# epfl-lts2/pygsp

Hardware: AMD Instinct MI355X
Metric: filtered-vertices/sec (N·Nsig·K/s) + achieved HBM GB/s vs roofline, 1M-vertex K=30 (higher is better)
Workload: dtype f64

## Files before the change

pygsp_amd/csrc/gspx.hip:

```cpp
#include "gspx_kernels.hip.h"
#include "gspx_tile_kernels.hip.h"

#include <hip/hip_runtime.h>

#include <algorithm>
#include <atomic>
#include <chrono>
#include <cmath>
#include <cstdarg>
#include <cstdio>
#include <cstring>
#include <map>
#include <memory>
#include <numeric>
#include <mutex>
#include <string>
#include <thread>
#include <vector>
#include <sys/mman.h>

#include "../../include/gspx.h"
#include "../../include/gspx_ext.h"

using namespace gspx;
// ... 292 lines not shown
  int64_t tile_pad = 1;
  int64_t tile_min_row = 16;
  int64_t staged_copy = 1;
  int64_t staged_copy_min_mb = 32;
  int64_t copy_threads = 0;
  int64_t tile_regroup = 1;
  int64_t tile_lg = 0;
  int64_t edge_vertex_walk = 1;
  int64_t fuse_input = 1;
  int64_t tile_nt = -1;
  int64_t synthesis = 0;
  int64_t alternate_sweep = 1;
  int64_t xcd_remap = 1;
  int64_t combine = 0;
  int64_t ws_limit_mb = 65536;
  int64_t max_batch = 0;
  int64_t gather_rccl = 1;
  int64_t lds_pad_kb = 0;
  int64_t host_pipeline = 1;
  int64_t host_batch = 0;
  int64_t host_edge = 0;
  int64_t host_threads = 0;
  int64_t streamed_alloc = 1;
};

struct gspx_ctx {
  int device = 0;
  int cu_count = 256;
  hipStream_t stream = nullptr;
  Options opt;
  DevMem ws_t;
  DevMem ws_r;
  DevMem ws_w;
  DevMem io_x, io_y;
  DevMem ws_spec;
  DevMem ws_sq, ws_sqp;
  HostPipe* pipe = nullptr;
  CopyStage* copy = nullptr;
  bool counted = false;
  std::mutex comms_mu;
  std::vector<struct gspx_comm*> comms;
  hipEvent_t ev[4] = {nullptr, nullptr, nullptr, nullptr};
  std::vector<hipEvent_t> ev_pool;
  double timing[8] = {0, 0, 0, 0, 0, 0, 0, 0};
  bool capturing = false;
  std::vector<unsigned char> seen_key;
  std::vector<unsigned char> graph_key;
  hipGraphExec_t graph_exec = nullptr;
};

static std::atomic<int> g_live_ctx[64];

static void replay_reset(gspx_ctx* ctx) {
  if (!ctx) return;
  ctx->seen_key.clear();
  ctx->graph_key.clear();
  if (ctx->graph_exec) {
    (void)hipGraphExecDestroy(ctx->graph_exec);
    ctx->graph_exec = nullptr;
  }
}

struct gspx_buf {
  gspx_ctx* ctx = nullptr;
  DevMem mem;
  int64_t bytes = 0;
// ... 86 lines not shown
    ctx->cu_count = 256;
  hipError_t e = hipStreamCreateWithFlags(&ctx->stream, hipStreamNonBlocking);
  if (e != hipSuccess) {
    delete ctx;
    return set_err(GSPX_ERR_HIP, "hipStreamCreate failed: %s", hipGetErrorString(e));
  }
  for (int i = 0; i < 4; ++i) {
    e = hipEventCreate(&ctx->ev[i]);
    if (e != hipSuccess) {
      delete ctx;
      return set_err(GSPX_ERR_HIP, "hipEventCreate failed: %s", hipGetErrorString(e));
    }
  }
  *out = ctx;
  return GSPX_OK;
}

static void comm_invalidate_all(gspx_ctx* ctx);

extern "C" int gspx_ctx_destroy(gspx_ctx* ctx) {
  replay_reset(ctx);
  if (!ctx) return GSPX_OK;
  if (ctx->counted) g_live_ctx[ctx->device & 63].fetch_sub(1);
  comm_invalidate_all(ctx);
  if (ctx->graph_exec) {
    (void)hipGraphExecDestroy(ctx->graph_exec);
    ctx->graph_exec = nullptr;
  }
  (void)hipSetDevice(ctx->device);
  if (ctx->stream) (void)hipStreamSynchronize(ctx->stream);
  for (int i = 0; i < 4; ++i)
    if (ctx->ev[i]) (void)hipEventDestroy(ctx->ev[i]);
  for (hipEvent_t e : ctx->ev_pool) (void)hipEventDestroy(e);
  ctx->ws_t.release();
  ctx->ws_r.release();
  ctx->ws_w.release();
  ctx->io_x.release();
  ctx->io_y.release();
  ctx->ws_spec.release();
  ctx->ws_sq.release();
  ctx->ws_sqp.release();
  if (ctx->pipe) {
    ctx->pipe->destroy();
    delete ctx->pipe;
    ctx->pipe = nullptr;
  }
  if (ctx->copy) {
    ctx->copy->destroy();
    delete ctx->copy;
    ctx->copy = nullptr;
  }
  if (ctx->stream) (void)hipStreamDestroy(ctx->stream);
  delete ctx;
  return GSPX_OK;
}

extern "C" int gspx_ctx_sync(gspx_ctx* ctx) {
  if (!ctx) return set_err(GSPX_ERR_INVALID, "null ctx");
  HIPCHK(hipSetDevice(ctx->device));
  HIPCHK(hipStreamSynchronize(ctx->stream));
  return GSPX_OK;
}

static int64_t* option_slot(Options& o, const char* key) {
  if (!key) return nullptr;
  if (!strcmp(key, "kernel")) return &o.kernel;
// ... 1039 lines not shown
}
static int sqnorm_gx(const gspx_ctx* ctx, int N, unsigned w) {
  const int cwl = sqnorm_cwl(w);
  const int64_t tiles = ((int64_t)N + (64 >> cwl) - 1) / (64 >> cwl);
  const int64_t gy = ((int64_t)w + (1 << cwl) - 1) >> cwl;
  return (int)std::max<int64_t>(1, std::min<int64_t>(tiles, (4 * (int64_t)ctx->cu_count + gy - 1) / gy));
}
static size_t sqnorm_parts(const gspx_ctx* ctx, int N, unsigned w) {
  return (size_t)sqnorm_gx(ctx, N, w) * SQ_PASS * w;
}

template <typename T>
static int launch_combine_sqnorm(gspx_ctx* ctx, const T* slots, int nslots, size_t slot_stride, unsigned pitch, int N,
                                 unsigned w, const SqNorms& sq, hipStream_t st) {
  const size_t lds = (size_t)nslots * 64 * sizeof(double);
  const int cwl = sqnorm_cwl(w);
  const dim3 grid((unsigned)sqnorm_gx(ctx, N, w), (w + (1u << cwl) - 1) >> cwl);
  for (int f0 = 0; f0 < sq.nf; f0 += SQ_PASS) {
    const int here = std::min(SQ_PASS, sq.nf - f0);
    const int fb = here <= 8 ? 2 : here <= 32 ? 8 : 32;
    typedef void (*kern_t)(const T*, int, size_t, u32, int, int, int, const double*, int, double*);
    const kern_t kern = fb == 2 ? k_combine_sqnorm<T, 2> : fb == 8 ? k_combine_sqnorm<T, 8> : k_combine_sqnorm<T, 32>;
    if (lds > ((size_t)64 << 10))
      HIPCHK(hipFuncSetAttribute((const void*)kern, hipFuncAttributeMaxDynamicSharedMemorySize, (int)lds));
    hipLaunchKernelGGL(kern, grid, dim3(256), lds, st, slots, nslots, slot_stride, (u32)pitch, N, (int)w, cwl,
                       sq.cf + f0, sq.ldc, sq.part);
    const int64_t n = (int64_t)here * w;
    hipLaunchKernelGGL(k_sqnorm_reduce, dim3((unsigned)((n + 255) / 256)), dim3(256), 0, st, sq.part, (int)grid.x,
                       4 * fb, here, (int)w, sq.out + (size_t)f0 * sq.ldo, sq.ldo);
  }
  return GSPX_OK;
}

template <typename T> static int ensure_factor(gspx_graph* g, double lmax) {
  if (g->fval_lmax == lmax) return GSPX_OK;
  gspx_ctx* ctx = g->ctx;
  const int N = (int)g->N;
  const T a1 = (T)(lmax / 2.0), a2 = (T)(lmax / 2.0);
  const T two_over_a1 = T(2) / a1;
  const int nb = std::max(1, (N + 255) / 256);
  if (N > 0)
    hipLaunchKernelGGL((k_factor<T>), dim3(nb), dim3(256), 0, ctx->stream, g->rptr.as<int>(),
                       g->rcol.as<int>(), g->rval.as<T>(), N, two_over_a1, a2, g->fval.as<T>());
  HIPCHK(hipGetLastError());
  g->fval_lmax = lmax;
  return GSPX_OK;
}

static hipEvent_t pool_event(gspx_ctx* ctx, size_t& i_ref) {
  size_t i = i_ref - 1;
  if (i >= 1024) {
    i = 1020 + (i & 3);
    i_ref = i + 1;
  }
  while (ctx->ev_pool.size() <= i) {
    hipEvent_t e = nullptr;
    if (hipEventCreate(&e) != hipSuccess) return nullptr;
    ctx->ev_pool.push_back(e);
  }
  return ctx->ev_pool[i];
}

__global__ void k_s1nat(const int* __restrict__ s1, const int* __restrict__ perm, int n, int* __restrict__ nat) {
  const int i = blockIdx.x * 256 + threadIdx.x;
  if (i < n) nat[i] = perm[s1[i]];
}
// ... 162 lines not shown
  a.perm = g->has_perm ? g->perm.as<int>() : nullptr;
  return a;
}

static int batch_events(gspx_ctx* ctx, size_t& ev_idx, hipEvent_t ev[4]) {
  for (int i = 0; i < 4; ++i) ev[i] = pool_event(ctx, ++ev_idx);
  if (!ev[0] || !ev[1] || !ev[2] || !ev[3]) return set_err(GSPX_ERR_HIP, "hipEventCreate failed");
  HIPCHK(hipEventRecord(ev[0], ctx->stream));
  return GSPX_OK;
}

template <typename T>
static int run_batch(gspx_graph* g, int nf, int M, const std::vector<double>& cp, const T* x,
                     unsigned ldx, T* y, unsigned ldy, unsigned ld, bool deferred,
                     bool acc_existing, bool final_to_y, size_t& ev_idx, const SqNorms* sq = nullptr) {
  gspx_ctx* ctx = g->ctx;
  const Options& opt = ctx->opt;
  hipStream_t st = ctx->stream;
  const int N = (int)g->N;
  const int K = M - 1;
  const WorkPanels wp = work_panels<T>(g, opt, deferred || nf == 1, 1, ld, y, ldy);
  const bool tile_direct = wp.tile_direct, padded = wp.padded;
  const unsigned ldw = wp.ldw;
  const size_t U = (size_t)N * ldw;
  const Shape shape = choose_shape(opt, sizeof(T), ld, vec_cap(4, ldy, y));
  const int* perm = g->has_perm ? g->perm.as<int>() : nullptr;

  std::vector<PlanStep> plan;
  if (deferred)
    make_plan_deferred(nf, M, plan);
  else
    make_plan_fused(nf, M, cp, acc_existing, final_to_y, plan);

  std::vector<T> hw;
  if (deferred) {
    hw.resize((size_t)nf * M);
    for (size_t i = 0; i < hw.size(); ++i) hw[i] = (T)cp[i];
  } else {
    hw.resize((size_t)K * nf * 3);
    for (int k = 0; k < K; ++k)
      for (int j = 0; j < nf * 3; ++j) hw[(size_t)k * nf * 3 + j] = (T)plan[(size_t)k].w[(size_t)j];
  }
  const bool cap = ctx->capturing;
  if (!cap) {
    CHK(ctx->ws_w.ensure(hw.size() * sizeof(T) + 64));
    HIPCHK(hipMemcpyAsync(ctx->ws_w.p, hw.data(), hw.size() * sizeof(T), hipMemcpyHostToDevice, st));
    HIPCHK(hipStreamSynchronize(st));
  }

  const size_t nslots = deferred ? (size_t)M : 2;
  const size_t SU = U;
  CHK(ctx->ws_t.ensure(nslots * SU * sizeof(T) + 256));
  if (!deferred) CHK(ctx->ws_r.ensure((size_t)nf * U * sizeof(T) + 256));
  T* slots = ctx->ws_t.as<T>();
  T* racc = ctx->ws_r.as<T>();

  hipEvent_t ev[4] = {};
  if (!cap) CHK(batch_events(ctx, ev_idx, ev));
  const bool tile_ok = tile_direct || padded;
  const unsigned char* xb = (const unsigned char*)x;
  const unsigned char* yb = (const unsigned char*)y;
  const size_t xbytes = (size_t)N * ldx * sizeof(T), ybytes = (size_t)nf * N * ldy * sizeof(T);
  const bool fuse_in = tile_direct && !deferred && opt.fuse_input && g->gt_slow == 0 && ldx == ld &&
                       ((uintptr_t)x % 16) == 0 && (xb + xbytes <= yb || yb + ybytes <= xb) &&
                       (!g->has_perm || (g->gt_ns1 > 0 && (!cap || g->gt_s1nat.p)));
  if (fuse_in) {
    CHK(ensure_s1nat(g, st));
  } else if (padded) {
    const unsigned nb = (unsigned)std::min<size_t>((U + 255) / 256, 65536);
    hipLaunchKernelGGL((k_permute_in_pad<T>), dim3(nb), dim3(256), 0, st, x, ldx, slots, ldw, ld, N, perm);
  } else {
    launch_permute_in<T>(x, ldx, slots, ld, N, perm, vec_cap(shape.vec, ldx, x), st);
  }
  if (!cap) HIPCHK(hipEventRecord(ev[1], st));

  CHK(prepare_coff<T>(g, shape, ld, st));
  StepArgs<T> a = step_base<T>(g, ld, y, ldy);
  a.nf = nf;
  a.racc = racc;
  for (int k = 1; k <= K; ++k) {
    const PlanStep& ps = plan[(size_t)k - 1];
    if (tile_ok) {
      TileArgs<T> t{};
      if (deferred) {
        t.cur = slots + (size_t)(k - 1) * SU;
        t.old = (k >= 2 && ps.gamma != 0.0) ? slots + (size_t)(k - 2) * SU : t.cur;
        t.out = slots + (size_t)k * SU;
      } else {
        t.cur = slots + (size_t)((k - 1) & 1) * SU;
        t.old = ps.gamma == 0.0 ? t.cur : slots + (size_t)(k & 1) * SU;
        t.out = slots + (size_t)(k & 1) * SU;
        if (fuse_in && k == 1) {
          t.cur = x;
          t.old = x;
          t.s1rows = g->has_perm ? g->gt_s1nat.as<int>() : nullptr;
        } else if (fuse_in && k == 2) {
          t.old = x;
          t.old_rows = perm;
        }
      }
      t.racc = racc;
      t.y = y;
      t.ldy = ldy;
      t.perm = perm;
      t.scale = (T)ps.scale;
      t.gamma = (T)ps.gamma;
      t.beta = T(0);
      t.flush = ps.flush;
      t.final = padded ? 0 : ps.final;
      t.reverse = (opt.alternate_sweep && (k & 1)) ? 1 : 0;
      if (ps.flush) {
        t.wn = (T)ps.w[0];
        t.wc = (T)ps.w[1];
        t.wo = (T)ps.w[2];
      }
      CHK(launch_step_tile<T>(g, opt, t, ldw, st));
      continue;
    }
    if (deferred) {
      a.cur = slots + (size_t)(k - 1) * SU;
      a.old = k >= 2 ? slots + (size_t)(k - 2) * SU : slots;
      a.out = slots + (size_t)k * SU;
    } else {
      a.cur = slots + (size_t)((k - 1) & 1) * SU;
      a.old = slots + (size_t)(k & 1) * SU;
      a.out = slots + (size_t)(k & 1) * SU;
    }
    if (ps.gamma == 0.0) a.old = a.cur;
    a.scale = (T)ps.scale;
    a.gamma = (T)ps.gamma;
    a.flush = ps.flush;
    a.final = ps.final;
    a.reverse = (opt.alternate_sweep && (k & 1)) ? 1 : 0;
    a.wts = ctx->ws_w.as<T>() + (size_t)(k - 1) * nf * 3;
    launch_step<T>(a, shape, opt, st, g->coff.as<unsigned>());
  }
  if (!cap) HIPCHK(hipEventRecord(ev[2], st));
  if (deferred && sq) {
    CHK(launch_combine_sqnorm<T>(ctx, slots, M, SU, ldw, N, ld, *sq, st));
  } else if (deferred) {
    launch_combine<T>(slots, M, SU, ctx->ws_w.as<T>(), M, nf, N, ld, y, ldy, (size_t)N * ldy, perm,
                      padded ? 1 : vec_cap(shape.vec, ldy, y), st, ldw);
  } else if (padded && final_to_y) {
    const unsigned nb = (unsigned)std::min<size_t>(((size_t)N * ld + 255) / 256, 65536);
    hipLaunchKernelGGL((k_permute_out_pad<T>), dim3(nb), dim3(256), 0, st, racc, ldw, y, ldy, ld, N, perm);
  }
  if (!cap) {
    HIPCHK(hipEventRecord(ev[3], st));
    HIPCHK(hipGetLastError());
  }
  return GSPX_OK;
}

template <typename T>
static int run_synthesis_batch(gspx_graph* g, int nf, int M, const std::vector<double>& cp,
                               const T* x, size_t plane_x, unsigned ldx, T* y, unsigned ldy,
                               unsigned ld, size_t& ev_idx);

static int batch_width(const gspx_graph* g, size_t elt, size_t panels, int64_t Nsig, int64_t* width) {
  const Options& opt = g->ctx->opt;
  const size_t rowb = (size_t)g->N * elt;
  int64_t max_ld = (int64_t)((((size_t)1 << 31) - 65536) / rowb);
  if (max_ld < 1)
    return set_err(GSPX_ERR_INVALID, "graph too large: one signal column exceeds 2 GiB");
  const size_t budget = (size_t)std::max<int64_t>(opt.ws_limit_mb, 1) << 20;
// ... 121 lines not shown
    if (analysis)
      return run_batch<T>(g, Nf, M, cp, x + c0, (unsigned)Nsig, y + c0, (unsigned)Nsig, ld, deferred, false, true,
                          ev_idx);
    if (opt.synthesis != 1)
      return run_synthesis_batch<T>(g, Nf, M, cp, x + c0, plane_x, (unsigned)Nsig, y + c0, (unsigned)Nsig, ld, ev_idx);
    for (int f = 0; f < Nf; ++f) {
      std::vector<double> cf(cp.begin() + (size_t)f * M, cp.begin() + (size_t)(f + 1) * M);
      CHK(run_batch<T>(g, 1, M, cf, x + (size_t)f * plane_x + c0, (unsigned)Nsig, y + c0, (unsigned)Nsig, ld, false,
                       f > 0, f == Nf - 1, ev_idx));
    }
    return GSPX_OK;
  });
}

template <typename T>
static int run_synthesis_batch(gspx_graph* g, int nf, int M, const std::vector<double>& cp,
                               const T* x, size_t plane_x, unsigned ldx, T* y, unsigned ldy,
                               unsigned ld, size_t& ev_idx) {
  gspx_ctx* ctx = g->ctx;
  Options opt = ctx->opt;
  hipStream_t st = ctx->stream;
  const int N = (int)g->N;
  const int K = M - 1;
  const WorkPanels wp = work_panels<T>(g, opt, true, (size_t)nf, ld, y, ldy);
  const bool padded = wp.padded;
  const unsigned ldw = wp.ldw;
  const size_t U = (size_t)N * ldw;
  const Shape shape = choose_shape(opt, sizeof(T), ld, vec_cap(4, ldy, y));
  const int* perm = g->has_perm ? g->perm.as<int>() : nullptr;

  std::vector<T> hw((size_t)M * nf);
  for (int k = 0; k < M; ++k)
    for (int f = 0; f < nf; ++f) hw[(size_t)k * nf + f] = (T)cp[(size_t)f * M + k];
  CHK(ctx->ws_w.ensure(hw.size() * sizeof(T) + 64));
  HIPCHK(hipMemcpyAsync(ctx->ws_w.p, hw.data(), hw.size() * sizeof(T), hipMemcpyHostToDevice, st));
  HIPCHK(hipStreamSynchronize(st));
  CHK(ctx->ws_r.ensure((size_t)nf * U * sizeof(T) + 256));
  CHK(ctx->ws_t.ensure(2 * U * sizeof(T) + 256));
  T* S = ctx->ws_r.as<T>();
  T* B[2] = {ctx->ws_t.as<T>(), ctx->ws_t.as<T>() + U};

  hipEvent_t ev[4];
  CHK(batch_events(ctx, ev_idx, ev));
  for (int f = 0; f < nf; ++f) {
    const T* xf = x + (size_t)f * plane_x;
    if (padded) {
      const unsigned nbp = (unsigned)std::min<size_t>((U + 255) / 256, 65536);
      hipLaunchKernelGGL((k_permute_in_pad<T>), dim3(nbp), dim3(256), 0, st, xf, ldx, S + (size_t)f * U, ldw, ld, N, perm);
      continue;
    }
    launch_permute_in<T>(xf, ldx, S + (size_t)f * U, ld, N, perm, vec_cap(shape.vec, ldx, xf), st);
  }
  HIPCHK(hipEventRecord(ev[1], st));

  CHK(prepare_coff<T>(g, shape, ld, st));
  StepArgs<T> a = step_base<T>(g, ld, y, ldy);
  a.nf = 1;
  a.nin = nf;
  a.racc = S;
  const bool tile_ok = wp.tile_direct || padded;
  for (int k = K; k >= 0; --k) {
    if (tile_ok) {
      TileArgs<T> t{};
      const bool has_b2 = (k + 2 <= K);
      t.cur = (k == K) ? S : B[(k + 1) & 1];
      t.old = (k < K && has_b2) ? B[k & 1] : t.cur;
      t.out = B[k & 1];
      t.racc = B[0];
      t.y = y;
// ... 22 lines not shown
      a.gamma = T(0);
    } else {
      a.cur = B[(k + 1) & 1];
      a.out = B[k & 1];
      const bool has_b2 = (k + 2 <= K);
      a.old = has_b2 ? B[k & 1] : a.cur;
      a.gamma = has_b2 ? T(-1) : T(0);
      a.scale = (k == 0) ? T(0.5) : T(1);
    }
    a.reverse = (opt.alternate_sweep && (k & 1)) ? 1 : 0;
    launch_step<T>(a, shape, opt, st, g->coff.as<unsigned>());
  }
  HIPCHK(hipEventRecord(ev[2], st));
  if (padded) {
    const unsigned nbp = (unsigned)std::min<size_t>(((size_t)N * ld + 255) / 256, 65536);
    hipLaunchKernelGGL((k_permute_out_pad<T>), dim3(nbp), dim3(256), 0, st, B[0], ldw, y, ldy, ld, N, perm);
  }
  HIPCHK(hipEventRecord(ev[3], st));
  HIPCHK(hipGetLastError());
  return GSPX_OK;
}

template <typename T>
static int run_program_batch(gspx_graph* g, int S, const double* sc, const double* be, const double* ga, bool old_is_x,
                             const T* x, unsigned ldx, T* y, unsigned ldy, unsigned ld, size_t& ev_idx) {
  gspx_ctx* ctx = g->ctx;
  Options opt = ctx->opt;
  hipStream_t st = ctx->stream;
  const int N = (int)g->N;
  const size_t U = (size_t)N * ld;
  const Shape shape = choose_shape(opt, sizeof(T), ld, vec_cap(4, ldy, y));
  const int* perm = g->has_perm ? g->perm.as<int>() : nullptr;

  const T hw[3] = {T(1), T(0), T(0)};
  CHK(ctx->ws_w.ensure(sizeof(hw) + 64));
  HIPCHK(hipMemcpyAsync(ctx->ws_w.p, hw, sizeof(hw), hipMemcpyHostToDevice, st));
  HIPCHK(hipStreamSynchronize(st));
  CHK(ctx->ws_t.ensure((old_is_x ? 3 : 2) * U * sizeof(T) + 256));
  T* X = ctx->ws_t.as<T>();
  T* H[2] = {X + U, old_is_x ? X + 2 * U : X};

  hipEvent_t ev[4];
  CHK(batch_events(ctx, ev_idx, ev));
  launch_permute_in<T>(x, ldx, X, ld, N, perm, vec_cap(shape.vec, ldx, x), st);
  HIPCHK(hipEventRecord(ev[1], st));

  CHK(prepare_coff<T>(g, shape, ld, st));
  StepArgs<T> a = step_base<T>(g, ld, y, ldy);
  a.nf = 1;
  a.racc = H[0];
  a.wts = ctx->ws_w.as<T>();
  const bool tile_ok = tile_usable<T>(g, opt, ld, y, ldy);
  for (int s = 0; s < S; ++s) {
    const bool last = s == S - 1;
    const T* cur = (s == 0) ? X : H[(s - 1) & 1];
    T* out = H[s & 1];
    const T* old = old_is_x ? X : (const T*)out;
    const double gam = (!old_is_x && s == 0) ? 0.0 : ga[s];
    if (tile_ok) {
      TileArgs<T> t{};
      t.cur = cur;
      t.old = gam == 0.0 ? cur : old;
      t.out = out;
      t.racc = H[0];
      t.y = y;
      t.ldy = ldy;
      t.perm = perm;
      t.scale = (T)sc[s];
      t.beta = (T)be[s];
      t.gamma = (T)gam;
      t.flush = 0;
      t.final = last ? 1 : 0;
      t.reverse = (opt.alternate_sweep && (s & 1)) ? 1 : 0;
      CHK(launch_step_tile<T>(g, opt, t, ld, st));
      continue;
    }
    a.cur = cur;
    a.old = gam == 0.0 ? cur : old;
    a.out = out;
    a.scale = (T)sc[s];
    a.beta = (T)be[s];
    a.gamma = (T)gam;
    a.flush = last ? 1 : 0;
    a.final = last ? 1 : 0;
    a.reverse = (opt.alternate_sweep && (s & 1)) ? 1 : 0;
    launch_step<T>(a, shape, opt, st, g->coff.as<unsigned>());
  }
  HIPCHK(hipEventRecord(ev[2], st));
  HIPCHK(hipEventRecord(ev[3], st));
  HIPCHK(hipGetLastError());
  return GSPX_OK;
}

template <typename T>
static int program_dev_t(gspx_graph* g, double lmax, int S, const double* sc, const double* be, const double* ga,
                         bool old_is_x, int64_t Nsig, const T* x, T* y) {
  gspx_ctx* ctx = g->ctx;
  replay_reset(ctx);
  for (int i = 0; i < 5; ++i) ctx->timing[i] = 0;
  if (g->N == 0 || Nsig == 0) return GSPX_OK;
  CHK(ensure_factor<T>(g, lmax));
  int64_t max_ld = 0;
  CHK(batch_width(g, sizeof(T), 3, Nsig, &max_ld));
  CHK(run_batches(g, Nsig, max_ld, S, [&](int64_t c0, unsigned ld, size_t& ev_idx) {
    return run_program_batch<T>(g, S, sc, be, ga, old_is_x, x + c0, (unsigned)Nsig, y + c0, (unsigned)Nsig, ld, ev_idx);
  }));
  ctx->timing[4] = 0;
  return GSPX_OK;
}

static void horner_program(int K, const double* nodes, const double* dc, std::vector<double>& sc,
                           std::vector<double>& be, std::vector<double>& ga) {
  sc.assign((size_t)K, 0.0);
  be.assign((size_t)K, 0.0);
  ga.assign((size_t)K, 0.0);
  for (int s = 0; s < K; ++s) {
    const int j = K - 1 - s;
// ... 670 lines not shown
```

pygsp_amd/csrc/gspx_kernels.hip.h:

```cpp
#pragma once
#include <hip/hip_runtime.h>
#include <stdint.h>

namespace gspx {

typedef unsigned int u32;
typedef u32 u32x2 __attribute__((ext_vector_type(2)));
typedef u32 u32x4 __attribute__((ext_vector_type(4)));
typedef __amdgpu_buffer_rsrc_t rsrc_t;

#ifndef GSPX_STREAM_AUX
#define GSPX_STREAM_AUX 0
#endif
#define GSPX_POISON 0x80000000u

template <typename T, int VEC> struct VT;

template <> struct VT<float, 1> {
  typedef float t;
  static __device__ __forceinline__ t bload(rsrc_t r, u32 o) {
    return __builtin_bit_cast(float, __builtin_amdgcn_raw_buffer_load_b32(r, o, 0, 0));
  }
  static __device__ __forceinline__ t sload(rsrc_t r, u32 o) {
    return __builtin_bit_cast(float, __builtin_amdgcn_raw_buffer_load_b32(r, o, 0, GSPX_STREAM_AUX));
// ... 64 lines not shown
  static __device__ __forceinline__ void sstore(rsrc_t r, u32 o, t v) {
    __builtin_amdgcn_raw_buffer_store_b128(__builtin_bit_cast(u32x4, v), r, o, 0, GSPX_STREAM_AUX);
  }
};

template <typename T> __device__ __forceinline__ T shfl_xor_t(T v, int off) { return __shfl_xor(v, off); }

template <typename T, int VEC>
__device__ __forceinline__ typename VT<T, VEC>::t vec_shfl_xor(typename VT<T, VEC>::t v, int off) {
  if constexpr (VEC == 1) {
    return __shfl_xor(v, off);
  } else {
    typename VT<T, VEC>::t o;
#pragma unroll
    for (int k = 0; k < VEC; ++k) o[k] = __shfl_xor(v[k], off);
    return o;
  }
}

template <typename T> struct StepArgs {
  const int* rowptr;
  const int* col;
  const T* val;
  const T* cur;
  const T* old;
  T* out;
  int N;
  u32 ld;
  u32 curbytes;
  T scale, gamma;
  T beta;
  int flush;
  int final;
  int nf;
  int nin;
  const T* wts;
  T* racc;
  T* y;
  u32 ldy;
  const int* perm;
  int rows_per_wave;
  int wpb;
  int lds_pad;
  int nchunks;
  int cpx;
  int reverse;
};

struct LaneSel {
  u32 m0, m1;
};
__device__ __forceinline__ LaneSel make_lane_sel(int r) {
  LaneSel s;
  s.m0 = (u32) - (r & 1);
  s.m1 = (u32) - ((r >> 1) & 1);
  asm volatile("" : "+v"(s.m0), "+v"(s.m1));
  return s;
}
__device__ __forceinline__ u32 blend(u32 a, u32 b, u32 m) { return a ^ ((a ^ b) & m); }
__device__ __forceinline__ int blend(int a, int b, u32 m) { return (int)blend((u32)a, (u32)b, m); }
__device__ __forceinline__ float blend(float a, float b, u32 m) {
  return __builtin_bit_cast(float, blend(__builtin_bit_cast(u32, a), __builtin_bit_cast(u32, b), m));
}
__device__ __forceinline__ double blend(double a, double b, u32 m) {
  const u32x2 ua = __builtin_bit_cast(u32x2, a), ub = __builtin_bit_cast(u32x2, b);
  u32x2 o;
// ... 188 lines not shown
                                                    const T* __restrict__ val,
                                                    const T* __restrict__ cur,
                                                    const T* __restrict__ wts,
                                                    const int* __restrict__ perm,
                                                    const StepArgs<T> a) {
  typedef typename VT<T, VEC>::t V;
  constexpr int W = 1 << WLOG2;
  constexpr int R = 64 / W;
  constexpr bool FLUSH = MODE == 1;

  const int lane = threadIdx.x & 63;
  const int wave = __builtin_amdgcn_readfirstlane(threadIdx.x >> 6);
  const int w = lane & (W - 1);

  int chunk = blockIdx.x;
  if (a.cpx > 0) chunk = (chunk & 7) * a.cpx + (chunk >> 3);
  if (chunk >= a.nchunks) return;
  if (a.reverse) chunk = a.nchunks - 1 - chunk;

  PanelCtx<T, VEC> c;
  c.rowptr = rowptr;
  c.col = col;
  c.val = val;
  c.wts = wts;
  c.perm = perm;
  c.r = lane >> WLOG2;
  c.sel = make_lane_sel(c.r);
  c.colel = (blockIdx.y * W + w) * VEC;
  c.lane_on = c.colel < a.ld;
  c.ldb = a.ld * (u32)sizeof(T);
  c.lane_off = c.lane_on ? c.colel * (u32)sizeof(T) : GSPX_POISON;
  c.rc = __builtin_amdgcn_make_buffer_rsrc((void*)cur, 0, a.curbytes, 0x00020000);
  c.rold = __builtin_amdgcn_make_buffer_rsrc((void*)a.old, 0, a.curbytes, 0x00020000);
  c.rout = __builtin_amdgcn_make_buffer_rsrc((void*)a.out, 0, a.curbytes, 0x00020000);
  c.rra = __builtin_amdgcn_make_buffer_rsrc((void*)a.racc, 0, a.curbytes, 0x00020000);
  c.row0 = (chunk * a.wpb + wave) * a.rows_per_wave;
  c.set_stride = R;
  c.nsets = a.rows_per_wave / R;

  if (c.row0 >= a.N) return;
  V ovA = 0, raA = 0, ovB = 0, raB = 0;
  {
    typedef VT<T, VEC> X;
    const int myrow = c.row0 + c.r;
    const u32 po = myrow < a.N ? (u32)myrow * c.ldb + c.lane_off : GSPX_POISON;
    ovA = X::sload(c.rold, po);
    if constexpr (FLUSH) raA = X::sload(c.rra, po);
  }
#pragma unroll 1
  for (int it = 0; it < c.nsets; it += 2) {
    if (!panel_row_set<T, VEC, R, MODE>(c, a, it, ovA, raA, ovB, raB)) break;
    if (it + 1 >= c.nsets) break;
    if (!panel_row_set<T, VEC, R, MODE>(c, a, it + 1, ovB, raB, ovA, raA)) break;
  }
}

template <typename T>
__global__ void k_coff(const int* __restrict__ rptr, const int* __restrict__ rcol, int N, u32 ldb,
                       u32* __restrict__ coff) {
  const int i = blockIdx.x * blockDim.x + threadIdx.x;
  if (i >= N) return;
  for (int j = rptr[i] & ~3; j < (rptr[i + 1] & ~3); ++j) {
    const int c = rcol[j];
    coff[j] = (c == N) ? GSPX_POISON : (u32)c * ldb;
  }
}

#define GSPX_LDS_CAP 512
// ... 157 lines not shown
                                                  const T* __restrict__ cur,
                                                  const T* __restrict__ wts,
                                                  const int* __restrict__ perm,
                                                  const StepArgs<T> a) {
  constexpr int W = 1 << WLOG2;
  constexpr int R = 64 / W;
  typedef T T4 __attribute__((ext_vector_type(4)));
  __shared__ u32x4 s_coff[4][GSPX_LDS_CAP / 4];
  __shared__ T4 s_val[4][GSPX_LDS_CAP / 4];

  const int lane = threadIdx.x & 63;
  const int wave = __builtin_amdgcn_readfirstlane(threadIdx.x >> 6);
  const int w = lane & (W - 1);

  int chunk = blockIdx.x;
  if (a.cpx > 0) chunk = (chunk & 7) * a.cpx + (chunk >> 3);
  if (chunk >= a.nchunks) return;
  if (a.reverse) chunk = a.nchunks - 1 - chunk;

  LdsCtx<T, VEC> c;
  c.s_coff = s_coff[wave];
  c.s_val = s_val[wave];
  c.coff = coff;
  c.val = val;
  c.wts = wts;
  c.perm = perm;
  c.r = lane >> WLOG2;
  c.colel = (blockIdx.y * W + w) * VEC;
  c.lane_on = c.colel < a.ld;
  c.ldb = a.ld * (u32)sizeof(T);
  c.lane_off = c.lane_on ? c.colel * (u32)sizeof(T) : GSPX_POISON;
  c.rc = __builtin_amdgcn_make_buffer_rsrc((void*)cur, 0, a.curbytes, 0x00020000);
  c.rold = __builtin_amdgcn_make_buffer_rsrc((void*)a.old, 0, a.curbytes, 0x00020000);
  c.rout = __builtin_amdgcn_make_buffer_rsrc((void*)a.out, 0, a.curbytes, 0x00020000);
  c.rra = __builtin_amdgcn_make_buffer_rsrc((void*)a.racc, 0, a.curbytes, 0x00020000);
  c.row0 = (chunk * 4 + wave) * a.rows_per_wave;
  if (c.row0 >= a.N) return;
  c.nsets = a.rows_per_wave / R;

  c.v_rp = rowptr[(c.row0 + lane) < a.N ? (c.row0 + lane) : a.N];
  c.seg_s = __builtin_amdgcn_readfirstlane(c.v_rp) & ~3;
  const int seg_e = __builtin_amdgcn_readlane(c.v_rp, a.rows_per_wave) & ~3;
  const int seg_n = seg_e - c.seg_s;

  if (seg_n <= GSPX_LDS_CAP) {
    for (int q = lane; q * 4 < seg_n; q += 64) {
      s_coff[wave][q] = *(const u32x4*)(coff + c.seg_s + 4 * q);
      s_val[wave][q] = *(const T4*)(val + c.seg_s + 4 * q);
    }
    lds_run_sets<T, VEC, R, MODE, true>(c, a);
  } else {
    lds_run_sets<T, VEC, R, MODE, false>(c, a);
  }
}

typedef unsigned short u16;
typedef unsigned char u8;

template <typename T, typename V, int LG = 16, typename I = u16>
__device__ __forceinline__ V lds_row_dot(const T* val, const I* idx, int len, const V* tile, int lane16,
                                         V& self) {
  typedef T T4 __attribute__((ext_vector_type(4)));
  typedef I I4 __attribute__((ext_vector_type(4)));
  V acc = 0;
  self = 0;
  for (int j = 0; j < len; j += 4) {
    const I4 ia = *(const I4*)(idx + j);
    const T4 va = *(const T4*)(val + j);
// ... 45 lines not shown
    T acc = 0;
    for (int j = s + g; j < e; j += 2 * G) {
      const int c0 = a.col[j];
      const T v0 = a.val[j];
      const int j1 = j + G;
      const bool on1 = j1 < e;
      const int c1 = on1 ? a.col[j1] : a.N;
      const T v1 = on1 ? a.val[j1] : T(0);
      const T x0 = X::bload(rc, (u32)c0 * ldb + lane_off);
      const T x1 = X::bload(rc, (u32)c1 * ldb + lane_off);
      acc += v0 * x0;
      acc += v1 * x1;
    }
    for (int off = W; off < (W << glog2); off <<= 1) acc += __shfl_xor(acc, off);

    if (row_on && g == 0 && lane_on) {
      const size_t o = (size_t)row * a.ld + w;
      T nv = a.scale * acc;
      T ov = 0;
      if (a.gamma != T(0)) {
        ov = a.old[o];
        nv += a.gamma * ov;
      }
      if (a.beta != T(0)) nv += a.beta * a.cur[o];
      if (!FLUSH && (a.nin > 0 || a.final)) {
        const size_t plane_in = (size_t)a.N * a.ld;
        for (int f = 0; f < a.nin; ++f) nv += a.wts[f] * a.racc[f * plane_in + o];
        if (a.final) {
          const size_t orow2 = a.perm ? (size_t)a.perm[row] : (size_t)row;
          a.y[orow2 * a.ldy + w] = nv;
          continue;
        }
      }
      a.out[o] = nv;
      if constexpr (FLUSH) {
        const T curv = a.cur[o];
        size_t orow = (size_t)row;
        if (a.final && a.perm) orow = (size_t)a.perm[row];
        const size_t plane_r = (size_t)a.N * a.ld;
        const size_t plane_y = (size_t)a.N * a.ldy;
        for (int f = 0; f < a.nf; ++f) {
          const T wn = a.wts[3 * f + 0], wc = a.wts[3 * f + 1], wo = a.wts[3 * f + 2];
          T r = wn * nv + wc * curv + wo * ov;
          if (a.flush == 2) r += a.racc[f * plane_r + o];
          if (a.final)
            a.y[f * plane_y + orow * a.ldy + w] = r;
          else
            a.racc[f * plane_r + o] = r;
        }
      }
    }
  }
}

template <typename T, int VEC, int NFB>
__global__ __launch_bounds__(256) void k_combine(const T* __restrict__ slots, int nslots,
                                                 size_t slot_stride, const T* __restrict__ cf,
                                                 int M, int f0, int nf_here, int N, u32 ld, T* y,
                                                 u32 ldy, size_t plane_y, const int* __restrict__ perm,
                                                 int accumulate, u32 pitch) {
  typedef typename VT<T, VEC>::t V;
  const u32 cpr = ld / VEC;
  const size_t total = (size_t)N * cpr;
  for (size_t idx = (size_t)blockIdx.x * 256 + threadIdx.x; idx < total;
       idx += (size_t)gridDim.x * 256) {
    const u32 row = (u32)(idx / cpr);
    const u32 ch = (u32)(idx - (size_t)row * cpr);
// ... 470 lines not shown
```

pygsp_amd/csrc/gspx_tile_kernels.hip.h:

```cpp
#pragma once

#include "gspx_kernels.hip.h"

namespace gspx {

template <typename T> struct TileArgs {
  const int* rowptr;
  const int* col;
  const T* val;
  const int* hdr;
  const int* s1rows;
  const u8* lidx;
  const T* cur;
  const T* old;
  const int* old_rows;
  T* out;
  T* racc;
  T* y;
  const int* perm;
  int N;
  u32 ld, ldy;
  u32 panel_bytes, val_bytes, lidx_bytes;
  int nb, ncol, per_xcd;
  int lds_bytes;
  T scale, gamma;
  T beta;
  T wn, wc, wo;
  const T* inp;
  const T* wts;
  int nin;
  int flush;
  int final;
  int reverse;
  int nt;
};

constexpr int GSPX_TILE_BR = 64;
constexpr int GSPX_TILE_MAXN1 = 160;

template <typename T, int NCOL, int LG, bool OLDNAT> struct TileSchedule {
  static constexpr bool PF = !OLDNAT;
  static constexpr bool TILE_LAST = PF && LG == 16;
  static constexpr bool PF_ENTRIES = PF;
  static constexpr bool META_AFTER = !OLDNAT && LG == 16 && NCOL == 0;
};

template <typename T, int NCOL, int LG = 16, bool OLDNAT = false, bool INS = false, int NT = 512, int CL = LG,
          int MIX = 0>
__global__ __launch_bounds__(NT, 4) void k_step_tile(const TileArgs<T> a) {
  static_assert(NT == 512 || (NT == 64 * LG && NCOL == 1) || (CL < LG && NCOL == 1 && NT % 64 == 0 && NT % CL == 0),
                "narrow builds: one row per group, one chunk per row");
  constexpr int BR = GSPX_TILE_BR;
  static_assert(CL <= LG && (BR % (NT / CL)) == 0, "compute groups must tile the block's rows");
  constexpr int MAXN1 = GSPX_TILE_MAXN1;
  constexpr bool PF = TileSchedule<T, NCOL, LG, OLDNAT>::PF;
  constexpr bool META_AFTER = TileSchedule<T, NCOL, LG, OLDNAT>::META_AFTER;
  constexpr bool TILE_LAST = TileSchedule<T, NCOL, LG, OLDNAT>::TILE_LAST;
  constexpr bool PF_ENTRIES = TileSchedule<T, NCOL, LG, OLDNAT>::PF_ENTRIES;
  constexpr int VEC = 16 / (int)sizeof(T);
  typedef typename VT<T, VEC>::t V;
  typedef __attribute__((address_space(3))) void* lds_ptr;
  extern __shared__ __attribute__((aligned(16))) unsigned char gspx_smem[];

  const int tid = threadIdx.x;
  constexpr int NGD = NT / LG;
// ... 201 lines not shown
          const int cc = a.col[j];
          const V xv = VT<T, VEC>::bload(rcur, cc < a.N ? (u32)cc * ldb + cb : POISON);
          if (j == s) self = xv;
          acc += a.val[j] * xv;
        }
      }
      nv[t] = a.scale * acc + a.gamma * ov[t] + a.beta * self;
      if constexpr (INS) nv[t] += ins[t];
      res[t] = a.wn * nv[t] + a.wc * self + a.wo * ov[t];
      if (a.flush == 2) res[t] += ra[t];
    }
    __builtin_amdgcn_s_waitcnt(0xC07F);
    if constexpr (MIX != 2) __builtin_amdgcn_s_barrier();
    bool more = true;
    if (last) {
      const int4 Hnn = uniform(Hv);
      H = Hn;
      Hn = Hnn;
      more = kn < k1;
    }
    __builtin_amdgcn_sched_barrier(0);
    if constexpr (!PF) {
      if (more && H.y >= 0) stage(M, H.y, chunk_off_d(last ? 0 : c + 1));
    }
#pragma unroll
    for (int t = 0; t < RPG; ++t) {
      const int row = row0 + t;
      if (row < a.N && on) {
        if (a.final && !a.flush) {
          const size_t orow = a.perm ? (size_t)a.perm[row] : (size_t)row;
          *(V*)(a.y + orow * a.ldy + col0) = nv[t];
          continue;
        }
        if (a.nt & 8) __builtin_nontemporal_store(nv[t], (V*)(a.out + (size_t)row * a.ld + col0));
        else *(V*)(a.out + (size_t)row * a.ld + col0) = nv[t];
        if (a.flush) {
          if (a.final) {
            const size_t orow = a.perm ? (size_t)a.perm[row] : (size_t)row;
            *(V*)(a.y + orow * a.ldy + col0) = res[t];
          } else {
            if (a.nt & 2) __builtin_nontemporal_store(res[t], (V*)(a.racc + (size_t)row * a.ld + col0));
            else *(V*)(a.racc + (size_t)row * a.ld + col0) = res[t];
          }
        }
      }
    }
    __builtin_amdgcn_sched_barrier(0);
    if constexpr (PF) {
      if (more) {
        const int nc = last ? 0 : c + 1;
        if constexpr (!TILE_LAST) {
          if (H.y >= 0) stage(M, H.y, chunk_off_d(nc));
        }
        prefetch_rows(M, last ? kn : k, nc);
        if constexpr (PF_ENTRIES) {
          if (last && H.y >= 0) prefetch_entries(H);
        }
        if constexpr (TILE_LAST) {
          __builtin_amdgcn_sched_barrier(0);
          if (H.y >= 0) stage(M, H.y, chunk_off_d(nc));
          __builtin_amdgcn_sched_barrier(0);
        }
      }
    }
    if (last) {
      k = kn;
      kn = knn;
      knn += nwx;
// ... 134 lines not shown
```

Before: 187.5 billion.

## Skip dead final-step output stores and redundant weight uploads with synchronous waits

Adds a drop_out flag so the last Chebyshev recurrence step stops writing its T_k output plane, which nothing reads afterward. Buffer resources for out and racc get zero size when unused, so those accesses become no-ops. Weight uploads now go through a cached pinned host buffer with an event, skipped when the contents are unchanged or the tile path does not use them, and the per-call hipStreamSynchronize is removed. This cuts one full N×ld store pass plus host sync latency, but relies on the output plane really being dead and on correct event handling for reuse of the pinned buffer.

```diff
diff --git a/pygsp_amd/csrc/gspx.hip b/pygsp_amd/csrc/gspx.hip
--- a/pygsp_amd/csrc/gspx.hip
+++ b/pygsp_amd/csrc/gspx.hip
@@ -348,6 +348,10 @@
   DevMem ws_t;
   DevMem ws_r;
   DevMem ws_w;
+  PinMem w_host;
+  size_t w_len = 0;
+  hipEvent_t w_ev = nullptr;
+  bool w_busy = false;
   DevMem io_x, io_y;
   DevMem ws_spec;
   DevMem ws_sq, ws_sqp;
@@ -500,6 +504,8 @@
   for (int i = 0; i < 4; ++i)
     if (ctx->ev[i]) (void)hipEventDestroy(ctx->ev[i]);
   for (hipEvent_t e : ctx->ev_pool) (void)hipEventDestroy(e);
+  if (ctx->w_ev) (void)hipEventDestroy(ctx->w_ev);
+  ctx->w_host.release();
   ctx->ws_t.release();
   ctx->ws_r.release();
   ctx->ws_w.release();
@@ -1605,6 +1611,26 @@
   return GSPX_OK;
 }
 
+static int upload_weights(gspx_ctx* ctx, const void* hw, size_t bytes) {
+  const void* const before = ctx->ws_w.p;
+  CHK(ctx->ws_w.ensure(bytes + 64));
+  if (ctx->ws_w.p != before) ctx->w_len = 0;
+  if (bytes == 0 || (ctx->w_len == bytes && !memcmp(ctx->w_host.p, hw, bytes))) return GSPX_OK;
+  if (ctx->w_busy) {
+    HIPCHK(hipEventSynchronize(ctx->w_ev));
+    ctx->w_busy = false;
+  }
+  ctx->w_len = 0;
+  CHK(ctx->w_host.ensure(std::max<size_t>(bytes, 4096)));
+  if (!ctx->w_ev) HIPCHK(hipEventCreateWithFlags(&ctx->w_ev, hipEventDisableTiming));
+  memcpy(ctx->w_host.p, hw, bytes);
+  HIPCHK(hipMemcpyAsync(ctx->ws_w.p, ctx->w_host.p, bytes, hipMemcpyHostToDevice, ctx->stream));
+  HIPCHK(hipEventRecord(ctx->w_ev, ctx->stream));
+  ctx->w_busy = true;
+  ctx->w_len = bytes;
+  return GSPX_OK;
+}
+
 template <typename T> static int ensure_factor(gspx_graph* g, double lmax) {
   if (g->fval_lmax == lmax) return GSPX_OK;
   gspx_ctx* ctx = g->ctx;
@@ -1833,20 +1859,19 @@
   else
     make_plan_fused(nf, M, cp, acc_existing, final_to_y, plan);
 
-  std::vector<T> hw;
-  if (deferred) {
-    hw.resize((size_t)nf * M);
-    for (size_t i = 0; i < hw.size(); ++i) hw[i] = (T)cp[i];
-  } else {
-    hw.resize((size_t)K * nf * 3);
-    for (int k = 0; k < K; ++k)
-      for (int j = 0; j < nf * 3; ++j) hw[(size_t)k * nf * 3 + j] = (T)plan[(size_t)k].w[(size_t)j];
-  }
+  const bool tile_ok = wp.tile_direct || wp.padded;
   const bool cap = ctx->capturing;
-  if (!cap) {
-    CHK(ctx->ws_w.ensure(hw.size() * sizeof(T) + 64));
-    HIPCHK(hipMemcpyAsync(ctx->ws_w.p, hw.data(), hw.size() * sizeof(T), hipMemcpyHostToDevice, st));
-    HIPCHK(hipStreamSynchronize(st));
+  if (!cap && (!tile_ok || (deferred && !sq))) {
+    std::vector<T> hw;
+    if (deferred) {
+      hw.resize((size_t)nf * M);
+      for (size_t i = 0; i < hw.size(); ++i) hw[i] = (T)cp[i];
+    } else {
+      hw.resize((size_t)K * nf * 3);
+      for (int k = 0; k < K; ++k)
+        for (int j = 0; j < nf * 3; ++j) hw[(size_t)k * nf * 3 + j] = (T)plan[(size_t)k].w[(size_t)j];
+    }
+    CHK(upload_weights(ctx, hw.data(), hw.size() * sizeof(T)));
   }
 
   const size_t nslots = deferred ? (size_t)M : 2;
@@ -1858,7 +1883,6 @@
 
   hipEvent_t ev[4] = {};
   if (!cap) CHK(batch_events(ctx, ev_idx, ev));
-  const bool tile_ok = tile_direct || padded;
   const unsigned char* xb = (const unsigned char*)x;
   const unsigned char* yb = (const unsigned char*)y;
   const size_t xbytes = (size_t)N * ldx * sizeof(T), ybytes = (size_t)nf * N * ldy * sizeof(T);
@@ -1909,6 +1933,7 @@
       t.beta = T(0);
       t.flush = ps.flush;
       t.final = padded ? 0 : ps.final;
+      t.drop_out = (!deferred && k == K) ? 1 : 0;
       t.reverse = (opt.alternate_sweep && (k & 1)) ? 1 : 0;
       if (ps.flush) {
         t.wn = (T)ps.w[0];
@@ -1932,6 +1957,7 @@
     a.gamma = (T)ps.gamma;
     a.flush = ps.flush;
     a.final = ps.final;
+    a.drop_out = (!deferred && k == K) ? 1 : 0;
     a.reverse = (opt.alternate_sweep && (k & 1)) ? 1 : 0;
     a.wts = ctx->ws_w.as<T>() + (size_t)(k - 1) * nf * 3;
     launch_step<T>(a, shape, opt, st, g->coff.as<unsigned>());
@@ -2119,9 +2145,7 @@
   std::vector<T> hw((size_t)M * nf);
   for (int k = 0; k < M; ++k)
     for (int f = 0; f < nf; ++f) hw[(size_t)k * nf + f] = (T)cp[(size_t)f * M + k];
-  CHK(ctx->ws_w.ensure(hw.size() * sizeof(T) + 64));
-  HIPCHK(hipMemcpyAsync(ctx->ws_w.p, hw.data(), hw.size() * sizeof(T), hipMemcpyHostToDevice, st));
-  HIPCHK(hipStreamSynchronize(st));
+  CHK(upload_weights(ctx, hw.data(), hw.size() * sizeof(T)));
   CHK(ctx->ws_r.ensure((size_t)nf * U * sizeof(T) + 256));
   CHK(ctx->ws_t.ensure(2 * U * sizeof(T) + 256));
   T* S = ctx->ws_r.as<T>();
@@ -2210,10 +2234,9 @@
   const Shape shape = choose_shape(opt, sizeof(T), ld, vec_cap(4, ldy, y));
   const int* perm = g->has_perm ? g->perm.as<int>() : nullptr;
 
+  const bool tile_ok = tile_usable<T>(g, opt, ld, y, ldy);
   const T hw[3] = {T(1), T(0), T(0)};
-  CHK(ctx->ws_w.ensure(sizeof(hw) + 64));
-  HIPCHK(hipMemcpyAsync(ctx->ws_w.p, hw, sizeof(hw), hipMemcpyHostToDevice, st));
-  HIPCHK(hipStreamSynchronize(st));
+  if (!tile_ok) CHK(upload_weights(ctx, hw, sizeof(hw)));
   CHK(ctx->ws_t.ensure((old_is_x ? 3 : 2) * U * sizeof(T) + 256));
   T* X = ctx->ws_t.as<T>();
   T* H[2] = {X + U, old_is_x ? X + 2 * U : X};
@@ -2228,7 +2251,6 @@
   a.nf = 1;
   a.racc = H[0];
   a.wts = ctx->ws_w.as<T>();
-  const bool tile_ok = tile_usable<T>(g, opt, ld, y, ldy);
   for (int s = 0; s < S; ++s) {
     const bool last = s == S - 1;
     const T* cur = (s == 0) ? X : H[(s - 1) & 1];
@@ -2261,6 +2283,7 @@
     a.gamma = (T)gam;
     a.flush = last ? 1 : 0;
     a.final = last ? 1 : 0;
+    a.drop_out = a.final;
     a.reverse = (opt.alternate_sweep && (s & 1)) ? 1 : 0;
     launch_step<T>(a, shape, opt, st, g->coff.as<unsigned>());
   }
diff --git a/pygsp_amd/csrc/gspx_kernels.hip.h b/pygsp_amd/csrc/gspx_kernels.hip.h
--- a/pygsp_amd/csrc/gspx_kernels.hip.h
+++ b/pygsp_amd/csrc/gspx_kernels.hip.h
@@ -120,6 +120,7 @@
   T beta;
   int flush;
   int final;
+  int drop_out;
   int nf;
   int nin;
   const T* wts;
@@ -374,8 +375,8 @@
   c.lane_off = c.lane_on ? c.colel * (u32)sizeof(T) : GSPX_POISON;
   c.rc = __builtin_amdgcn_make_buffer_rsrc((void*)cur, 0, a.curbytes, 0x00020000);
   c.rold = __builtin_amdgcn_make_buffer_rsrc((void*)a.old, 0, a.curbytes, 0x00020000);
-  c.rout = __builtin_amdgcn_make_buffer_rsrc((void*)a.out, 0, a.curbytes, 0x00020000);
-  c.rra = __builtin_amdgcn_make_buffer_rsrc((void*)a.racc, 0, a.curbytes, 0x00020000);
+  c.rout = __builtin_amdgcn_make_buffer_rsrc((void*)a.out, 0, a.drop_out ? 0u : a.curbytes, 0x00020000);
+  c.rra = __builtin_amdgcn_make_buffer_rsrc((void*)a.racc, 0, a.flush == 2 ? a.curbytes : 0u, 0x00020000);
   c.row0 = (chunk * a.wpb + wave) * a.rows_per_wave;
   c.set_stride = R;
   c.nsets = a.rows_per_wave / R;
@@ -599,8 +600,8 @@
   c.lane_off = c.lane_on ? c.colel * (u32)sizeof(T) : GSPX_POISON;
   c.rc = __builtin_amdgcn_make_buffer_rsrc((void*)cur, 0, a.curbytes, 0x00020000);
   c.rold = __builtin_amdgcn_make_buffer_rsrc((void*)a.old, 0, a.curbytes, 0x00020000);
-  c.rout = __builtin_amdgcn_make_buffer_rsrc((void*)a.out, 0, a.curbytes, 0x00020000);
-  c.rra = __builtin_amdgcn_make_buffer_rsrc((void*)a.racc, 0, a.curbytes, 0x00020000);
+  c.rout = __builtin_amdgcn_make_buffer_rsrc((void*)a.out, 0, a.drop_out ? 0u : a.curbytes, 0x00020000);
+  c.rra = __builtin_amdgcn_make_buffer_rsrc((void*)a.racc, 0, a.flush == 2 ? a.curbytes : 0u, 0x00020000);
   c.row0 = (chunk * 4 + wave) * a.rows_per_wave;
   if (c.row0 >= a.N) return;
   c.nsets = a.rows_per_wave / R;
@@ -712,7 +713,7 @@
           continue;
         }
       }
-      a.out[o] = nv;
+      if (!a.drop_out) a.out[o] = nv;
       if constexpr (FLUSH) {
         const T curv = a.cur[o];
         size_t orow = (size_t)row;
diff --git a/pygsp_amd/csrc/gspx_tile_kernels.hip.h b/pygsp_amd/csrc/gspx_tile_kernels.hip.h
--- a/pygsp_amd/csrc/gspx_tile_kernels.hip.h
+++ b/pygsp_amd/csrc/gspx_tile_kernels.hip.h
@@ -31,6 +31,7 @@
   int nin;
   int flush;
   int final;
+  int drop_out;
   int reverse;
   int nt;
 };
@@ -298,8 +299,10 @@
           *(V*)(a.y + orow * a.ldy + col0) = nv[t];
           continue;
         }
-        if (a.nt & 8) __builtin_nontemporal_store(nv[t], (V*)(a.out + (size_t)row * a.ld + col0));
-        else *(V*)(a.out + (size_t)row * a.ld + col0) = nv[t];
+        if (!a.drop_out) {
+          if (a.nt & 8) __builtin_nontemporal_store(nv[t], (V*)(a.out + (size_t)row * a.ld + col0));
+          else *(V*)(a.out + (size_t)row * a.ld + col0) = nv[t];
+        }
         if (a.flush) {
           if (a.final) {
             const size_t orow = a.perm ? (size_t)a.perm[row] : (size_t)row;
```

Result: no change. 188.5 billion, median of 6 (+0.5%).
